# SEpapoulis/ODElib

Measured on AMD Instinct MI355X. Metric: walker-timesteps/sec, 4-state infection ODE, 65536 walkers, 1/2/4/8 MI355X, higher is better.
Workload: dtype f64

## Files before the change

### odelib_amd/csrc/capi.hip

```cpp
#include <hip/hip_runtime.h>

#include <algorithm>
#include <array>
#include <cstdlib>
#include <memory>
#include <mutex>
#include <cmath>
#include <cstdio>
#include <cstring>
#include <new>
#include <string>
#include <vector>

#include "../../include/odelib_amd.h"
#include "aux_kernels.h"
#include "dispatch.h"
#include "launch_plan.h"
#include "rtc.h"

#define OE_BUILTINS(X) \
  X(zero_i) X(one_i) X(two_i) X(chain4) X(chain5) X(chain6) X(chain8) X(chain10) X(chain12) X(chain16) X(chain20) \
  X(chain24) X(chain32)
#define X(NAME) OE_DECLARE_ENTRY(NAME);
OE_BUILTINS(X)
// ... 378 lines not shown
      if (b->p) (void)hipFree(b->p);
    if (c->ev0) (void)hipEventDestroy(c->ev0);
    if (c->ev1) (void)hipEventDestroy(c->ev1);
    if (c->np_stream) {
      (void)hipStreamSynchronize(c->np_stream);
      (void)hipStreamDestroy(c->np_stream);
    }
    for (int k = 0; k < 2; ++k) {
      if (c->ev_np[k]) (void)hipEventDestroy(c->ev_np[k]);
      if (c->ev_mh[k]) (void)hipEventDestroy(c->ev_mh[k]);
    }
    for (auto& m : c->custom)
      for (hipModule_t md : {m->rtc.mod, m->rtc.stiff_mod})
        if (md) (void)hipModuleUnload(md);
    (void)hipStreamDestroy(c->own_stream);
  }
  delete c;
}

const char* oe_last_error(const oe_ctx* c) {
  if (c) return c->err.c_str();
  return g_err.empty() ? "null context" : g_err.c_str();
}

int oe_rtc_check(const char* rhs_body, int32_t n_states, int32_t n_params, const char* arch) {
  if (!rhs_body || n_states < 1 || n_states > 64 || n_params < 1 || n_params > 60)
    return fail(nullptr, OE_ERR_ARG, "oe_rtc_check: bad arguments");
  std::string err;
  if (rtc_build(rhs_body, n_states, n_params, arch ? arch : "gfx950", kRtcExplicit, nullptr, nullptr, err))
    return fail(nullptr, OE_ERR_ARG, err);
  g_err.clear();
  return OE_OK;
}

int oe_model_compile(oe_ctx* c, const char* rhs_body, int32_t n_states, int32_t n_params, int32_t* model_id) {
  if (!c || !c->own_stream) return OE_ERR_STATE;
  if (!rhs_body || !model_id || n_states < 1 || n_states > 64 || n_params < 1 || n_params > 60)
    return fail(c, OE_ERR_ARG, "oe_model_compile: bad arguments");
  for (size_t k = 0; k < c->custom.size(); ++k) {
    const CustomModel& m = *c->custom[k];
    if (m.body == rhs_body && m.entry.S == n_states && m.entry.P == n_params) {
      *model_id = OE_MODEL_CUSTOM + (int32_t)k;
      return OE_OK;
    }
  }
  OE_DEVICE_GUARD(c);
  auto m = std::make_unique<CustomModel>();
  std::string err;
  if (rtc_build(rhs_body, n_states, n_params, c->arch.c_str(), kRtcExplicit, &m->rtc, &m->entry, err))
    return fail(c, OE_ERR_ARG, err);
  m->body = rhs_body;
  m->entry.model_id = OE_MODEL_CUSTOM + (int32_t)c->custom.size();
  m->entry.S = n_states;
  m->entry.P = n_params;
  *model_id = m->entry.model_id;
  c->custom.push_back(std::move(m));
  return OE_OK;
}

int oe_ctx_set_stream(oe_ctx* c, void* s) {
  if (!c || !c->own_stream) return OE_ERR_STATE;
  c->stream = static_cast<hipStream_t>(s);
  return OE_OK;
}

int oe_ctx_use_own_stream(oe_ctx* c) {
  if (!c || !c->own_stream) return OE_ERR_STATE;
  c->stream = c->own_stream;
  return OE_OK;
}

int oe_problem_set(oe_ctx* c, const oe_problem* p) {
  if (!c || !c->own_stream) return OE_ERR_STATE;
  if (!p) return fail(c, OE_ERR_ARG, "oe_problem_set: null problem");
  OE_DEVICE_GUARD(c);
  const Entry* e = nullptr;
  CustomModel* cm = nullptr;
  if (p->model_id >= OE_MODEL_CUSTOM) {
    const size_t k = (size_t)(p->model_id - OE_MODEL_CUSTOM);
    if (k < c->custom.size()) {
      cm = c->custom[k].get();
      e = &cm->entry;
    }
  } else {
    e = find_entry(p->model_id, p->n_states);
  }
  if (!e)
    return fail(c, OE_ERR_UNSUPPORTED, "oe_problem_set: model " + std::to_string(p->model_id) +
                                           " with S=" + std::to_string(p->n_states) +
                                           " is not compiled in");
  if (p->n_states != e->S) return fail(c, OE_ERR_ARG, "oe_problem_set: n_states mismatch");
  const int pmax = e->P + (e->S < 4 ? e->S : 4);
  if (p->n_params < e->P || p->n_params > pmax)
    return fail(c, OE_ERR_ARG, "oe_problem_set: n_params must be in [model P, model P + min(S, 4)]");
  if (p->n_times < 2 || !p->times) return fail(c, OE_ERR_ARG, "oe_problem_set: need >= 2 times");
  for (int i = 1; i < p->n_times; ++i)
    if (!(p->times[i] > p->times[i - 1]))
      return fail(c, OE_ERR_ARG, "oe_problem_set: times must be strictly increasing");
  if (p->method < OE_METHOD_RK4 || p->method > OE_METHOD_BDF)
    return fail(c, OE_ERR_ARG, "oe_problem_set: unknown method");
  if (p->method == OE_METHOD_BDF && e->S > kStiffRegS)
    return fail(c, OE_ERR_UNSUPPORTED, "oe_problem_set: bdf needs n_states <= " + std::to_string(kStiffRegS));
  if (p->method == OE_METHOD_AUTO || p->method == OE_METHOD_ROSENBROCK || p->method == OE_METHOD_BDF) {
    if (cm) {
      if (cm->rtc.stiff == 0) {
        std::string err;
        if (rtc_build(cm->body, e->S, e->P, c->arch.c_str(), kRtcStiff, &cm->rtc, &cm->entry, err)) {
          cm->rtc.stiff = -1;
          cm->rtc.stiff_err = err;
        }
      }
      if (cm->rtc.stiff != 1) return fail(c, OE_ERR_UNSUPPORTED, "oe_problem_set: " + cm->rtc.stiff_err);
    } else if (!e->integrate[p->method][0][0] && !(p->method == OE_METHOD_AUTO && e->integrate_hq[0][0][0])) {
      return fail(c, OE_ERR_UNSUPPORTED, "oe_problem_set: the stiff methods (auto, rosenbrock) need n_states <= " +
                                             std::to_string(kStiffMaxS));
    }
  }
  if (p->method == OE_METHOD_RK4 && p->rk4_substeps < 1)
    return fail(c, OE_ERR_ARG, "oe_problem_set: rk4_substeps must be >= 1");
  if (p->method != OE_METHOD_RK4 &&
      (!(p->rtol > 0.0) || !(p->atol >= 0.0) || p->max_steps < 2))
    return fail(c, OE_ERR_ARG, "oe_problem_set: adaptive methods need rtol > 0, atol >= 0, max_steps >= 2");
  if (p->n_obs < 0) return fail(c, OE_ERR_ARG, "oe_problem_set: n_obs < 0");
  if (p->n_obs > 0 && (!p->obs_tidx || !p->obs_mask || !p->obs_log || !p->obs_logsigma || !p->obs_lin))
    return fail(c, OE_ERR_ARG, "oe_problem_set: observation arrays missing");

  std::vector<Obs> obs_in(p->n_obs);
  const uint64_t valid_mask = (e->S >= 64) ? ~0ull : ((1ull << e->S) - 1ull);
  for (int k = 0; k < p->n_obs; ++k) {
    if (p->obs_tidx[k] < 0 || p->obs_tidx[k] >= p->n_times)
      return fail(c, OE_ERR_ARG, "oe_problem_set: obs_tidx out of range");
    if (p->obs_mask[k] == 0 || (p->obs_mask[k] & ~valid_mask))
      return fail(c, OE_ERR_ARG, "oe_problem_set: obs_mask selects no / unknown states");
    Obs& o = obs_in[k];
    o.tidx = p->obs_tidx[k];
    o.pad = 0;
    o.mask = p->obs_mask[k];
    o.O = p->obs_log[k];
    const double s = p->obs_logsigma[k];
    o.two_s2 = 2.0 * (s * s);
    o.O_lin = p->obs_lin[k];
  }
  std::vector<int32_t> perm(p->n_obs);
  for (int k = 0; k < p->n_obs; ++k) perm[k] = k;
  std::stable_sort(perm.begin(), perm.end(), [&](int32_t a, int32_t b) { return obs_in[a].tidx < obs_in[b].tidx; });
  std::vector<Obs> obs(p->n_obs);
  std::vector<double> c_rec(p->n_obs);
  for (int k = 0; k < p->n_obs; ++k) {
    obs[k] = obs_in[perm[k]];
    c_rec[k] = -(std::log(p->obs_logsigma[perm[k]]) + 0.5 * std::log(2.0 * 3.14159265358979323846));
  }

  const int nsub = p->method == OE_METHOD_RK4 ? p->rk4_substeps : 1;
  std::vector<double> rk4(4 * (size_t)p->n_times);
  for (int i = 1; i < p->n_times; ++i) {
    const double h = (p->times[i] - p->times[i - 1]) / (double)nsub;
    rk4[4 * (i - 1)] = h;
    rk4[4 * (i - 1) + 1] = 0.5 * h;
    rk4[4 * (i - 1) + 2] = h / 6.0;
    rk4[4 * (i - 1) + 3] = p->times[i - 1];
  }
  for (int j = 0; j < 4; ++j) rk4[4 * (size_t)(p->n_times - 1) + j] = rk4[4 * (size_t)(p->n_times - 2) + j];

  OE_HIP(c, hipStreamSynchronize(c->stream));
  if (c->d_times) { OE_HIP(c, hipFree(c->d_times)); c->d_times = nullptr; }
  if (c->d_obs) { OE_HIP(c, hipFree(c->d_obs)); c->d_obs = nullptr; }
  if (c->d_rk4) { OE_HIP(c, hipFree(c->d_rk4)); c->d_rk4 = nullptr; }
  OE_HIP(c, hipMalloc(&c->d_rk4, sizeof(double) * rk4.size()));
  OE_HIP(c, hipMemcpy(c->d_rk4, rk4.data(), sizeof(double) * rk4.size(), hipMemcpyHostToDevice));
  std::vector<double> tg(p->times, p->times + p->n_times);
  tg.insert(tg.end(), oe::kGridWin + 1, HUGE_VAL);
  OE_HIP(c, hipMalloc(&c->d_times, sizeof(double) * tg.size()));
  OE_HIP(c, hipMemcpy(c->d_times, tg.data(), sizeof(double) * tg.size(), hipMemcpyHostToDevice));
  if (p->n_obs > 0) {
    OE_HIP(c, hipMalloc(&c->d_obs, sizeof(Obs) * p->n_obs));
    OE_HIP(c, hipMemcpy(c->d_obs, obs.data(), sizeof(Obs) * p->n_obs, hipMemcpyHostToDevice));
  }
  DevProblem& d = c->dp;
  d.times = c->d_times;
  d.rk4 = c->d_rk4;
  d.obs = c->d_obs;
  d.T = p->n_times;
  d.n_obs = p->n_obs;
  d.P = p->n_params;
  d.substeps = p->method == OE_METHOD_RK4 ? p->rk4_substeps : 1;
  d.rtol = p->rtol;
  d.atol = p->atol;
  d.max_steps = p->max_steps;
  d.pnum = p->pnum;
  d.sstot = p->sstot;
  d.newton_tol = std::fmax(10.0 * 2.220446049250313e-16 / p->rtol, std::fmin(0.03, std::sqrt(p->rtol)));
  c->method = p->method;
  c->entry = e;
  c->has_problem = true;
  c->band_cols = c->band_bins = 0;
  c->waic_on = false;
  c->waic_c = std::move(c_rec);
  c->waic_perm = std::move(perm);
  c->err.clear();
  return OE_OK;
}

int oe_integrate(oe_ctx* c, int64_t W, const double* y0, const double* theta, double* traj,
                 double* chi, double* ssres, int32_t* status, uint32_t flags) {
  if (!c || !c->own_stream) return OE_ERR_STATE;
  if (!c->has_problem) return fail(c, OE_ERR_STATE, "oe_integrate: call oe_problem_set first");
  if (W <= 0 || W > kMaxWalkers) return fail(c, OE_ERR_ARG, "oe_integrate: n_walkers must be in [1, 2^29]");
  if (!y0 || !theta) return fail(c, OE_ERR_ARG, "oe_integrate: y0 and theta are required");
  OE_DEVICE_GUARD(c);
  int rc = OE_OK;
  const Entry* e = c->entry;
  const int S = e->S, P = c->dp.P, T = c->dp.T;
  const bool host = flags & OE_HOST_PTRS;
  const bool nt = flags & OE_NT_STORES;
  if (traj && (int64_t)S * W * 8 >= (int64_t(1) << 32))
    return fail(c, OE_ERR_ARG, "oe_integrate: one trajectory row (S*W*8 bytes) must be < 4 GiB");

  IntegrateArgs ia{};
  ia.W = W;
  if (host) {
    const size_t n_in = (size_t)(S + P) * W;
    const size_t n_traj = traj ? (size_t)T * S * W : 0;
    const size_t n_out = (size_t)2 * W;
    const size_t bytes = sizeof(double) * (n_in + n_traj + n_out) + sizeof(int32_t) * W + 256;
    rc = c->scratch.reserve(c, bytes);
    if (rc) return rc;
    double* base = static_cast<double*>(c->scratch.p);
    double* d_y0 = base;
    double* d_th = d_y0 + (size_t)S * W;
    double* d_traj = traj ? d_th + (size_t)P * W : nullptr;
    double* d_chi = d_th + (size_t)P * W + n_traj;
    double* d_ss = d_chi + W;
    int32_t* d_st = reinterpret_cast<int32_t*>(d_ss + W);
    OE_HIP(c, hipMemcpyAsync(d_y0, y0, sizeof(double) * S * W, hipMemcpyHostToDevice, c->stream));
    OE_HIP(c, hipMemcpyAsync(d_th, theta, sizeof(double) * P * W, hipMemcpyHostToDevice, c->stream));
    ia.y0 = d_y0; ia.theta = d_th; ia.traj = d_traj; ia.chi = d_chi; ia.ssres = d_ss; ia.status = d_st;
  } else {
    ia.y0 = y0; ia.theta = theta; ia.traj = traj; ia.chi = chi; ia.ssres = ssres; ia.status = status;
  }
  const plan::ModelCaps caps = caps_of(e, P);
  plan::IntegratePlan pl =
      plan::plan_integrate(caps, c->method, W, c->n_cu, ia.traj != nullptr, nt, flags, xcd_run_walkers());
  c->dp.obs_c = nullptr;
  if (pl.obs_scratch && c->dp.n_obs > 0) {
    rc = c->obs.reserve(c, sizeof(double) * (size_t)c->dp.n_obs * (size_t)W);
    if (rc) return rc;
    c->dp.obs_c = static_cast<double*>(c->obs.p);
  }
  c->has_last_tune = false;
  if (pl.path == plan::kRk4Traj && (flags & OE_TUNE)) {
    rc = tune_rk4(c, e, caps, ia, nt, flags, pl, &c->last_tune);
    if (rc) return rc;
    plan::shape_rk4_traj(pl, c->last_tune.variant, W, flags, xcd_run_walkers());
    c->has_last_tune = true;
  }
  c->last_variant = pl.variant;
  c->hq_ctl = nullptr;
  ia.half = pl.half;
  ia.xcd_remap = pl.xcd_remap;
  const int tj = ia.traj ? 1 : 0, nj = nt ? 1 : 0;
  const bool wave_stiff = pl.path == plan::kDirectWaveStiff || pl.path == plan::kWaveStiff;
  StiffWaveArgs sa{};
  int32_t* stiff_buf = nullptr;
  if (wave_stiff) {
    rc = c->stiff.reserve(c, sizeof(int32_t) * (size_t)(2 * W + 64));
    if (rc) return rc;
    stiff_buf = static_cast<int32_t*>(c->stiff.p);
    sa.y0 = ia.y0; sa.theta = ia.theta; sa.traj = ia.traj; sa.chi = ia.chi; sa.ssres = ia.ssres; sa.W = W;
    if (!ia.status) ia.status = stiff_buf + 64 + W;
    sa.status = ia.status;
  }
  const bool timing = !(flags & OE_NO_TIMING);
  if (timing) OE_HIP(c, hipEventRecord(c->ev0, c->stream));
  if (pl.path == plan::kHandQueue) {
    HandQ q{};
    rc = ensure_hq(c, W, S, &q);
    if (rc) return rc;
    q.n_waves = (int32_t)pl.grid * (kBlock / 64);
    OE_HIP(c, hipMemsetAsync(q.ctl, 0, 10 * sizeof(int32_t), c->stream));
    hipStream_t bs = c->stream;
    if (pl.beside) {
      OE_HIP(c, hipEventRecord(c->ev_hq[0], c->stream));
      OE_HIP(c, hipStreamWaitEvent(c->hq_stream, c->ev_hq[0], 0));
      bs = c->hq_stream;
    }
    const int bj = pl.beside ? 1 : 0;
    OE_HIP(c, launch(e->integrate_hq[bj][tj][nj], dim3(pl.grid), dim3(pl.block), c->stream, c->dp, ia, q));
    OE_HIP(c, launch(e->bdf_hq[bj][tj][nj], dim3(pl.G), dim3(64), bs, c->dp, ia, q));
    if (pl.beside) {
      OE_HIP(c, hipEventRecord(c->ev_hq[1], c->hq_stream));
      OE_HIP(c, hipStreamWaitEvent(c->stream, c->ev_hq[1], 0));
    }
    c->hq_ctl = q.ctl;
  } else if (pl.path != plan::kWaveStiff) {
    OE_HIP(c, launch_planned(c, e, pl, ia, nt));
  }
  if (wave_stiff) {
    if (pl.path == plan::kDirectWaveStiff) {
      int32_t* count = stiff_buf;
      int32_t* list = stiff_buf + 64;
      OE_HIP(c, hipMemsetAsync(count, 0, sizeof(int32_t), c->stream));
      OE_HIP(c, launch(kernel_of(k_stiff_list), dim3((unsigned)((W + 255) / 256)), dim3(256), c->stream,
                       (const int32_t*)ia.status, W, list, count));
      sa.list = list;
      sa.count = count;
    }
    OE_HIP(c, launch(e->stiff_wave[tj][nj], dim3(pl.wave_grid), dim3(64), c->stream, c->dp, sa));
  }
  OE_HIP(c, hipGetLastError());
  if (timing) OE_HIP(c, hipEventRecord(c->ev1, c->stream));
  c->timed = timing;

  if (host) {
    if (traj)
      OE_HIP(c, hipMemcpyAsync(traj, ia.traj, sizeof(double) * T * S * W, hipMemcpyDeviceToHost, c->stream));
// ... 572 lines not shown
```

### odelib_amd/csrc/ode_kernels.cuh

```cuda
#pragma once
#include <hip/hip_runtime.h>
#include <stdint.h>
#include "models.cuh"

namespace oe {

struct Obs {
  int32_t tidx;
  int32_t pad;
  uint64_t mask;
  double O;
  double two_s2;
  double O_lin;
};

template <class T>
using cptr = const __attribute__((address_space(4))) T*;
template <class T>
__device__ __forceinline__ cptr<T> kconst(const T* p) {
  return (cptr<T>)(p);
}

struct DevProblem {
  const double* times;
// ... 117 lines not shown

typedef unsigned int u32x2 __attribute__((ext_vector_type(2)));
typedef unsigned int u32x4 __attribute__((ext_vector_type(4)));

#ifndef OE_NT_AUX
#define OE_NT_AUX 18
#endif
template <bool NT>
__device__ __forceinline__ void st_row(__amdgpu_buffer_rsrc_t rsrc, uint32_t lane_off, uint32_t s_off, double v) {
  __builtin_amdgcn_raw_buffer_store_b64(__builtin_bit_cast(u32x2, v), rsrc, lane_off, s_off, NT ? OE_NT_AUX : 0);
}

#ifndef OE_TRANSC_CALL
#define OE_TRANSC_CALL 1
#endif
#if OE_TRANSC_CALL
__device__ __attribute__((noinline)) double oe_log(double x) { return log(x); }
__device__ __attribute__((noinline)) double oe_exp(double x) { return exp(x); }
#else
__device__ __forceinline__ double oe_log(double x) { return log(x); }
__device__ __forceinline__ double oe_exp(double x) { return exp(x); }
#endif

template <int S>
__device__ __forceinline__ void check_finite(const double (&y)[S], Acc& a) {
#pragma unroll
  for (int s = 0; s < S; ++s) a.nf = fma(y[s], 0.0, a.nf);
}

template <int S>
__device__ __forceinline__ void track_min(const double (&y)[S], Acc& a) {
  if constexpr (S == 1) {
    a.ymin = min_raw(a.ymin, y[0]);
  } else {
    double m[(S + 1) / 2];
#pragma unroll
    for (int j = 0; j < S / 2; ++j) m[j] = min_raw(y[2 * j], y[2 * j + 1]);
    if constexpr (S % 2) m[S / 2] = y[S - 1];
    double r = m[0];
#pragma unroll
    for (int j = 1; j < (S + 1) / 2; ++j) r = min_raw(r, m[j]);
    a.ymin = min_raw(a.ymin, r);
  }
}

template <int S, bool TRAJ, bool NT>
__device__ __forceinline__ void store_row_at(double* row, const double (&y)[S], int64_t W, uint32_t off,
                                             bool active, Acc& a) {
  track_min<S>(y, a);
  if constexpr (TRAJ) {
    if (active) {
      const uint32_t row_bytes = (uint32_t)(S * W * 8);
      const __amdgpu_buffer_rsrc_t rsrc = __builtin_amdgcn_make_buffer_rsrc((void*)row, 0, row_bytes, 0x00020000);
#pragma unroll
      for (int s = 0; s < S; ++s) st_row<NT>(rsrc, off, (uint32_t)(s * W * 8), y[s]);
    }
  }
}

template <int S, bool TRAJ, bool NT>
__device__ __forceinline__ void store_row(int i, const double (&y)[S], double* __restrict__ traj,
                                          int64_t W, uint32_t off, bool active, Acc& a) {
  store_row_at<S, TRAJ, NT>(TRAJ ? traj + (int64_t)i * S * W : nullptr, y, W, off, active, a);
}

struct ObsTerm { double O, two_s2, O_lin; };
template <class ObsPtr>
__device__ __forceinline__ ObsTerm obs_term(ObsPtr rec) {
  return ObsTerm{rec->O, rec->two_s2, rec->O_lin};
}
template <int S>
__device__ __forceinline__ double masked_sum(const double (&y)[S], uint64_t mask) {
  double c = 0.0;
#pragma unroll
  for (int s = 0; s < S; ++s)
    if ((mask >> s) & 1ull) c = c + y[s];
  return c;
}
template <bool INLINE_LOG = false>
__device__ __forceinline__ double chi_term(const ObsTerm& t, double c) {
  const double d = t.O - (INLINE_LOG ? log(c) : oe_log(c));
  return (d * d) / t.two_s2;
}
template <bool INLINE_LOG = false>
__device__ __forceinline__ void fold_obs(const ObsTerm& t, double c, Acc& a, bool in = true) {
  const double term = chi_term<INLINE_LOG>(t, c);
  if (in && __builtin_isfinite(term)) { a.chi += term; a.nvalid += 1; }
  const double r = c - t.O_lin;
  const double r2 = r * r;
  if (in && !__builtin_isnan(r2)) a.ssres += r2;
}
template <class ObsPtr>
__device__ __forceinline__ int next_observed(const DevProblem& pb, ObsPtr obs, int k) {
  return (k < pb.n_obs) ? obs[k].tidx : 0x7fffffff;
}

template <int S, bool INLINE_LOG = false>
__device__ __forceinline__ void observe(const DevProblem& pb, int i, const double (&y)[S], int& k, Acc& a) {
  const cptr<Obs> obs = kconst(pb.obs);
  if (!(k < pb.n_obs && obs[k].tidx == i)) return;
  check_finite(y, a);
  for (; k < pb.n_obs && obs[k].tidx == i; ++k) {
    const uint64_t mask = obs[k].mask;
    const ObsTerm rec = obs_term(obs + k);
    double c = 0.0;
#pragma unroll
    for (int s = 0; s < S; ++s)
      if ((mask >> s) & 1ull) c = c + y[s];
    fold_obs<INLINE_LOG>(rec, c, a);
  }
}

template <int S>
__device__ __forceinline__ void observe_next(const DevProblem& pb, int i, const double (&y)[S], int& k,
                                             int& nxt, Acc& a) {
  if (i != nxt) return;
  observe<S>(pb, i, y, k, a);
  nxt = next_observed(pb, kconst(pb.obs), k);
}

template <int S, bool TRAJ, bool NT, bool INLINE_LOG = false>
__device__ __forceinline__ void emit(const DevProblem& pb, int i, const double (&y)[S],
                                     double* __restrict__ traj, int64_t W, uint32_t off,
                                     bool active, int& k, Acc& a) {
  store_row<S, TRAJ, NT>(i, y, traj, W, off, active, a);
  observe<S, INLINE_LOG>(pb, i, y, k, a);
}

template <int S, bool TRAJ>
__device__ __forceinline__ bool grid_needs_emit(const DevProblem& pb, int i, int k) {
  if constexpr (TRAJ) return true;
  return k < pb.n_obs && kconst(pb.obs)[k].tidx == i;
}

template <class M, int PMAX>
__device__ __forceinline__ void rk4_step(double (&y)[M::S], double t, double h, double hh, double h6,
                                         const double (&p)[PMAX]) {
  constexpr int S = M::S;
  double k[S], acc[S], yt[S];
  M::rhs(y, t, p, k);
#pragma unroll
  for (int s = 0; s < S; ++s) { acc[s] = k[s]; yt[s] = fma(hh, k[s], y[s]); }
  M::rhs(yt, t + hh, p, k);
#pragma unroll
  for (int s = 0; s < S; ++s) { acc[s] = fma(2.0, k[s], acc[s]); yt[s] = fma(hh, k[s], y[s]); }
  M::rhs(yt, t + hh, p, k);
#pragma unroll
  for (int s = 0; s < S; ++s) { acc[s] = fma(2.0, k[s], acc[s]); yt[s] = fma(h, k[s], y[s]); }
  M::rhs(yt, t + h, p, k);
#pragma unroll
  for (int s = 0; s < S; ++s) { acc[s] = acc[s] + k[s]; y[s] = fma(h6, acc[s], y[s]); }
}

template <class M, int PMAX, bool TRAJ, bool NT>
__device__ __forceinline__ void integrate_rk4(const DevProblem& pb, double (&y)[M::S],
                                              const double (&p)[PMAX], double* traj,
                                              int64_t W, uint32_t off, bool active, Acc& a) {
  constexpr int S = M::S;
  int k = 0;
  emit<S, TRAJ, NT, TRAJ>(pb, 0, y, traj, W, off, active, k, a);
  const int n = pb.substeps;
  const cptr<Obs> obs = kconst(pb.obs);
  cptr<double> tab = kconst(pb.rk4);
  double h = tab[0], hh = tab[1], h6 = tab[2], t = tab[3];
  tab += 4;
  double* trow = TRAJ ? traj + (int64_t)S * W : nullptr;
  auto interval = [&]() {
    const double hn = tab[0], hhn = tab[1], h6n = tab[2], tn = tab[3];
    tab += 4;
    for (int j = 0; j < n; ++j) rk4_step<M, PMAX>(y, t + (double)j * h, h, hh, h6, p);
    h = hn; hh = hhn; h6 = h6n; t = tn;
  };
  int i = 1;
  while (i < pb.T) {
    const int next = (k < pb.n_obs) ? obs[k].tidx : pb.T;
    for (; i < next; ++i) {
      interval();
      if constexpr (TRAJ) {
        store_row_at<S, TRAJ, NT>(trow, y, W, off, active, a);
        trow += S * W;
      }
    }
    if (i < pb.T) {
      interval();
      store_row_at<S, TRAJ, NT>(trow, y, W, off, active, a);
      if constexpr (TRAJ) trow += S * W;
      observe<S, TRAJ>(pb, i, y, k, a);
      ++i;
    }
  }
  check_finite(y, a);
}

namespace dp {
constexpr double c2 = 1.0 / 5, c3 = 3.0 / 10, c4 = 4.0 / 5, c5 = 8.0 / 9;
constexpr double a21 = 1.0 / 5;
constexpr double a31 = 3.0 / 40, a32 = 9.0 / 40;
constexpr double a41 = 44.0 / 45, a42 = -56.0 / 15, a43 = 32.0 / 9;
constexpr double a51 = 19372.0 / 6561, a52 = -25360.0 / 2187, a53 = 64448.0 / 6561,
                 a54 = -212.0 / 729;
constexpr double a61 = 9017.0 / 3168, a62 = -355.0 / 33, a63 = 46732.0 / 5247,
                 a64 = 49.0 / 176, a65 = -5103.0 / 18656;
constexpr double a71 = 35.0 / 384, a73 = 500.0 / 1113, a74 = 125.0 / 192,
                 a75 = -2187.0 / 6784, a76 = 11.0 / 84;
constexpr double e1 = 71.0 / 57600, e3 = -71.0 / 16695, e4 = 71.0 / 1920,
                 e5 = -17253.0 / 339200, e6 = 22.0 / 525, e7 = -1.0 / 40;
constexpr double d1 = -12715105075.0 / 11282082432.0, d3 = 87487479700.0 / 32700410799.0,
                 d4 = -10690763975.0 / 1880347072.0, d5 = 701980252875.0 / 199316789632.0,
                 d6 = -1453857185.0 / 822651844.0, d7 = 69997945.0 / 29380423.0;
constexpr double safe = 0.9, facmin = 0.2, facmax = 10.0;

__device__ const double kTab[36] = {a21, a31, a32, a41, a42, a43, a51, a52, a53, a54, a61, a62, a63, a64, a65,
                                    a71, a73, a74, a75, a76, e1, e3, e4, e5, e6, e7, d1, d3, d4, d5, d6, d7,
                                    c2, c3, c4, c5};
constexpr double kTabC[36] = {a21, a31, a32, a41, a42, a43, a51, a52, a53, a54, a61, a62, a63, a64, a65,
                              a71, a73, a74, a75, a76, e1, e3, e4, e5, e6, e7, d1, d3, d4, d5, d6, d7,
                              c2, c3, c4, c5};
struct Tab {
  double v[36];
};
template <bool VREG, bool MIX = false, bool PIN = false>
__device__ __forceinline__ Tab load_tab() {
  Tab t;
  if constexpr (VREG) {
    int z;
    asm volatile("v_mov_b32 %0, 0" : "=v"(z));
    const double* p = kTab + z;
#pragma unroll
    for (int j = 0; j < 36; ++j) t.v[j] = (MIX && j >= 20) ? kTabC[j] : p[j];
  } else {
    const double c[36] = {a21, a31, a32, a41, a42, a43, a51, a52, a53, a54, a61, a62, a63, a64, a65,
                          a71, a73, a74, a75, a76, e1, e3, e4, e5, e6, e7, d1, d3, d4, d5, d6, d7,
                          c2, c3, c4, c5};
#pragma unroll
    for (int j = 0; j < 36; ++j) {
      if constexpr (PIN) {
        constexpr uint64_t kOne = 1;
        const uint64_t b = __builtin_bit_cast(uint64_t, c[j]);
        uint32_t lo, hi;
        asm volatile("s_mov_b32 %0, %2\n\ts_mov_b32 %1, %3" : "=s"(lo), "=s"(hi)
                     : "i"((uint32_t)(b & 0xffffffffu)), "i"((uint32_t)(b >> 32)));
        (void)kOne;
        t.v[j] = __builtin_bit_cast(double, ((uint64_t)hi << 32) | lo);
      } else {
        t.v[j] = c[j];
      }
    }
  }
  return t;
}

template <int N>
__device__ __forceinline__ double select_r(int r, const double (&c)[N]) {
  static_assert(N >= 1 && N <= 8, "select_r: at most 8 entries");
  auto at = [&](int k) { return c[k < N ? k : N - 1]; };
  const bool b0 = (r & 1) != 0, b1 = (r & 2) != 0, b2 = (r & 4) != 0;
  const double l0 = b0 ? at(1) : at(0), l1 = b0 ? at(3) : at(2);
  const double l2 = b0 ? at(5) : at(4), l3 = b0 ? at(7) : at(6);
  const double m0 = b1 ? l1 : l0, m1 = b1 ? l3 : l2;
  return b2 ? m1 : m0;
}

template <int N>
__device__ __forceinline__ int count_le(const double (&w)[N], double x) {
  int c = 0;
#pragma unroll
  for (int j = 0; j < N; ++j) {
    c += (w[j] <= x) ? 1 : 0;
    asm("" : "+v"(c));
  }
  return c;
}

__device__ __forceinline__ double inv_fifth_root(double x) {
  int e;
  const double m = frexp(x, &e);
  int q = e / 5, r = e % 5;
  if (r < 0) { r += 5; q -= 1; }
  double y = fma(fma(0.2395, m, -0.6505), m, 1.4123);
#pragma unroll
  for (int it = 0; it < 2; ++it) {
    const double y2 = y * y;
    const double y5 = (y2 * y2) * y;
    y = (y * fma(-m, y5, 6.0)) * 0.2;
  }
  constexpr double kC[5] = {1.0, 0.8705505632961241, 0.757858283255199, 0.6597539553864471, 0.5743491774985174};
  return ldexp(select_r(r, kC) * y, -q);
}

constexpr int kFifthBias = 1088;
struct FifthScale {
  double v[2 * kFifthBias];
  constexpr FifthScale() : v() {
    const double c[5] = {1.0, 0.8705505632961241, 0.757858283255199, 0.6597539553864471, 0.5743491774985174};
    for (int j = 0; j < 2 * kFifthBias; ++j) {
      const int e = j - kFifthBias;
      int q = e / 5, r = e % 5;
      if (r < 0) { r += 5; q -= 1; }
      const int be = 1023 - q;
      v[j] = (be > 0 && be < 2047) ? c[r] * __builtin_bit_cast(double, (unsigned long long)be << 52) : 0.0;
    }
  }
};
__device__ const FifthScale kFifthScale{};
__device__ __forceinline__ double inv_fifth_root_uniform(double x, cptr<double> scale) {
  int e;
  const double m = frexp(x, &e);
  e = __builtin_amdgcn_readfirstlane(e);
  const double sc = scale[e + kFifthBias];
  double y = fma(fma(0.2395, m, -0.6505), m, 1.4123);
#pragma unroll
  for (int it = 0; it < 2; ++it) {
    const double y2 = y * y;
    const double y5 = (y2 * y2) * y;
    y = (y * fma(-m, y5, 6.0)) * 0.2;
  }
  return sc * y;
}
}

constexpr int kDpPipeFields = 6;
template <int S>
constexpr int dp_pipe_slots() {
  return (150 * 1024) / (4 * (kDpPipeFields * S * 64 * 8 + 32)) < 8 ? (150 * 1024) / (4 * (kDpPipeFields * S * 64 * 8 + 32)) : 8;
}
template <int S>
struct DpPipe {
  double* ring;
  double* uni;
  volatile int* produced;
  volatile int* consumed;
  int lane, R, n, cons_seen;
};

__device__ __forceinline__ void lds_fence() { asm volatile("s_waitcnt lgkmcnt(0)" ::: "memory"); }

template <int S>
__device__ __forceinline__ void dp_pipe_publish(DpPipe<S>& pp, double t, double tn, double rh, const double (&y)[S],
                                                const double (&ydf)[S], const double (&bsp)[S], const double (&r4)[S],
                                                const double (&r5)[S], const double (&yn)[S]) {
  while (pp.n - pp.cons_seen >= pp.R) {
    pp.cons_seen = *pp.consumed;
    if (pp.n - pp.cons_seen >= pp.R) __builtin_amdgcn_s_sleep(1);
// ... 616 lines not shown
#pragma unroll
  for (int q = 0; q < PMAX; ++q) p[q] = (q < pb.P) ? ia.theta[(int64_t)q * W + w] : 0.0;
#if OE_HQ_TRACE
  const uint64_t t_claim = __builtin_amdgcn_s_memrealtime();
#endif
  if (OE_HQ_PRIO) __builtin_amdgcn_s_setprio(3);
  integrate_bdf_lane<M, PMAX, TRAJ, NT, DREG ? 0 : 64>(pb, y, t, i, k, p, ia.traj, W, w, part, part, a);
#if OE_HQ_TRACE
  {
    const uint64_t t0 = __hip_atomic_load((const uint64_t*)(hq.ctl + 4 + 2), __ATOMIC_RELAXED, __HIP_MEMORY_SCOPE_AGENT);
    const uint64_t t_pend = __hip_atomic_load((const uint64_t*)(hq.ctl + 8), __ATOMIC_RELAXED, __HIP_MEMORY_SCOPE_AGENT);
    a.chi = (double)((int64_t)(t_start - t0) / 100) * 1e5 + (double)((int64_t)(t_pend - t0) / 100);
    a.ssres = (double)((int64_t)(t_claim - t0) / 100) * 1e5 + (double)((__builtin_amdgcn_s_memrealtime() - t_claim) / 100);
    a.nvalid = 1;
  }
#endif
  if (part) {
    if (ia.chi) ia.chi[w] = a.nvalid ? a.chi : __builtin_nan("");
    if (ia.ssres) ia.ssres[w] = a.ssres;
    if (ia.status) ia.status[w] = finish(a);
  }
}

template <class M, bool NT>
__global__ void __launch_bounds__(512) k_integrate_dopri5_piped(const DevProblem pb, const IntegrateArgs ia) {
  constexpr int S = M::S;
  constexpr int PMAX = kPmax<M>;
  constexpr int R = dp_pipe_slots<S>();
  static_assert(R >= 2, "slot ring too small");
  __shared__ double ring[4][R][kDpPipeFields * S * 64];
  __shared__ double uni[4][R][4];
  __shared__ int produced[4], consumed[4];
  __shared__ double ymin_sh[4][64];
  const int wave = threadIdx.x >> 6;
  const int lane = threadIdx.x & 63;
  const int c = wave & 3;
  if (threadIdx.x < 4) { produced[threadIdx.x] = 0; consumed[threadIdx.x] = 0; }
  __syncthreads();
  const int64_t blk = ia.xcd_remap ? xcd_block(blockIdx.x, gridDim.x, ia.xcd_remap) : (int64_t)blockIdx.x;
  const int64_t gw = blk * 256 + c * 64 + lane;
  const bool active = gw < ia.W;
  const int64_t w = active ? gw : ia.W - 1;
  const int64_t W = ia.W;
  const int T = pb.T;
  if (wave < 4) {
    double y[S], p[PMAX];
#pragma unroll
    for (int s = 0; s < S; ++s) y[s] = ia.y0[(int64_t)s * W + w];
#pragma unroll
    for (int j = 0; j < PMAX; ++j) p[j] = (j < pb.P) ? ia.theta[(int64_t)j * W + w] : 0.0;
    Acc a = acc_init();
    DpPipe<S> pp{&ring[c][0][0], &uni[c][0][0], &produced[c], &consumed[c], lane, R, 0, 0};
    integrate_dopri5<M, PMAX, true, NT, false, false, false, true>(pb, y, p, ia.traj, W, (uint32_t)w * 8u, active, a,
                                                                 nullptr, &pp);
    __syncthreads();
    a.ymin = min_raw(a.ymin, ymin_sh[c][lane]);
    if (active) {
      if (ia.chi) ia.chi[w] = a.nvalid ? a.chi : __builtin_nan("");
      if (ia.ssres) ia.ssres[w] = a.ssres;
      if (ia.status) ia.status[w] = finish(a);
    }
  } else {
    const double* times = pb.times;
    const uint32_t off = (uint32_t)w * 8u;
    const uint32_t row_bytes = (uint32_t)(S * W * 8);
    Acc a = acc_init();
    int i = 0;
    for (int n = 0; i < T; ++n) {
      while (*(volatile int*)&produced[c] <= n) __builtin_amdgcn_s_sleep(1);
      asm volatile("" ::: "memory");
      const int slot = n % R;
      const double* f = &ring[c][slot][0] + lane;
      const double t = uni[c][slot][0], tn = uni[c][slot][1], rh = uni[c][slot][2];
      double y[S], ydf[S], bsp[S], r4[S], r5[S], yn[S];
#pragma unroll
      for (int s = 0; s < S; ++s) {
        y[s] = f[(0 * S + s) * 64];
        ydf[s] = f[(1 * S + s) * 64];
        bsp[s] = f[(2 * S + s) * 64];
        r4[s] = f[(3 * S + s) * 64];
        r5[s] = f[(4 * S + s) * 64];
        yn[s] = f[(5 * S + s) * 64];
      }
      lds_fence();
      if (lane == 0) *(volatile int*)&consumed[c] = n + 1;
      double ti = times[i];
      while (ti < tn) {
        const double th = (ti - t) * rh;
        const double th1 = 1.0 - th;
        double yo[S];
#pragma unroll
        for (int s = 0; s < S; ++s)
          yo[s] = fma(th, fma(th1, fma(th, fma(th1, r5[s], r4[s]), bsp[s]), ydf[s]), y[s]);
        store_row_at<S, true, NT>(ia.traj + (int64_t)i * S * W, yo, W, off, active, a);
        ++i;
        ti = times[i];
      }
      if (i < T && ti == tn) {
        store_row_at<S, true, NT>(ia.traj + (int64_t)i * S * W, yn, W, off, active, a);
        ++i;
      }
    }
    (void)row_bytes;
    ymin_sh[c][lane] = a.ymin;
    __syncthreads();
  }
}

constexpr int kPipeWalkers = 256;
#ifndef OE_PIPE_LDS_BYTES
#define OE_PIPE_LDS_BYTES (160 * 1024)
#endif
constexpr int kPipeLdsBytes = OE_PIPE_LDS_BYTES;

template <int S>
constexpr int pipe_rows() { return (kPipeLdsBytes / (2 * S * kPipeWalkers * 8)) > 0 ? (kPipeLdsBytes / (2 * S * kPipeWalkers * 8)) : 1; }

__device__ __forceinline__ void lds_barrier() {
  asm volatile("s_waitcnt lgkmcnt(0)" ::: "memory");
  __builtin_amdgcn_s_barrier();
  asm volatile("" ::: "memory");
}


template <class M, bool NT, int NSW>
__global__ void __launch_bounds__(256 + 64 * NSW) k_integrate_rk4_piped(const DevProblem pb, const IntegrateArgs ia) {
  constexpr int S = M::S;
  constexpr int PMAX = kPmax<M>;
  constexpr int H = pipe_rows<S>();
  static_assert(2 * H * S * kPipeWalkers * 8 <= kPipeLdsBytes, "LDS ring too large");
  __shared__ double pipe_ring[2][H][S][kPipeWalkers];
  auto ring = [&](int half, int h, int s, int b) -> double* { return &pipe_ring[half][h][s][b]; };

  const int64_t W = ia.W;
  const int T = pb.T;
  const int wave = threadIdx.x >> 6;
  const int lane = threadIdx.x & 63;
  const int64_t blk = ia.xcd_remap ? xcd_block(blockIdx.x, gridDim.x, ia.xcd_remap) : (int64_t)blockIdx.x;
  const int64_t base = blk * kPipeWalkers;
  const int nphase = (T + H - 1) / H;

  if (wave < 4) {
    const int b = wave * 64 + lane;
    const int64_t gw = base + b;
    const bool active = gw < W;
    const int64_t w = active ? gw : W - 1;
    double y[S], p[PMAX];
#pragma unroll
    for (int s = 0; s < S; ++s) y[s] = ia.y0[(int64_t)s * W + w];
#pragma unroll
    for (int j = 0; j < PMAX; ++j) p[j] = (j < pb.P) ? ia.theta[(int64_t)j * W + w] : 0.0;
    Acc a = acc_init();
    int k = 0;
    const cptr<double> tab = kconst(pb.rk4);
    const cptr<Obs> obs = kconst(pb.obs);
    const int n = pb.substeps;
    auto put = [&](int half, int h, const double (&v)[S]) {
#pragma unroll
      for (int s = 0; s < S; ++s) *ring(half, h, s, b) = v[s];
#pragma unroll
      for (int s = 0; s < S; ++s) a.ymin = min_raw(a.ymin, v[s]);
    };
    auto interval = [&](int i) {
      const double h = tab[4 * (i - 1)], hh = tab[4 * (i - 1) + 1], h6 = tab[4 * (i - 1) + 2];
      const double t = tab[4 * (i - 1) + 3];
      for (int j = 0; j < n; ++j) rk4_step<M, PMAX>(y, t + (double)j * h, h, hh, h6, p);
    };
    for (int ph = 0; ph <= nphase; ++ph) {
      if (ph < nphase) {
        const int half = ph & 1;
        const int r0 = ph * H;
        const int r1 = (r0 + H < T) ? r0 + H : T;
        int r = r0;
        if (r == 0) {
          put(half, 0, y);
          observe<S, true>(pb, 0, y, k, a);
          ++r;
        }
        while (r < r1) {
          int next = (k < pb.n_obs) ? obs[k].tidx : T;
          if (next > r1) next = r1;
          for (; r < next; ++r) {
            interval(r);
            put(half, r - r0, y);
          }
          if (r < r1) {
            interval(r);
            put(half, r - r0, y);
            observe<S, true>(pb, r, y, k, a);
            ++r;
          }
        }
      }
      lds_barrier();
    }
    check_finite(y, a);
    if (active) {
      if (ia.chi) ia.chi[w] = a.nvalid ? a.chi : __builtin_nan("");
      if (ia.ssres) ia.ssres[w] = a.ssres;
      if (ia.status) ia.status[w] = finish(a);
    }
  } else {
    const int sw = wave - 4;
    constexpr int G = NSW / 2;
    const int sg = sw >> 1;
    const int b = (sw & 1) * 128 + 2 * lane;
    const bool active = base + b < W;
    const uint32_t off = (uint32_t)(base + b) * 8u;
    const uint32_t row_bytes = (uint32_t)(S * W * 8);
    for (int ph = 0; ph <= nphase; ++ph) {
      if (ph >= 1) {
        const int half = (ph - 1) & 1;
        const int r0 = (ph - 1) * H;
        const int r1 = (r0 + H < T) ? r0 + H : T;
        for (int r = r0; r < r1; ++r) {
          const __amdgpu_buffer_rsrc_t rsrc =
              __builtin_amdgcn_make_buffer_rsrc((void*)(ia.traj + (int64_t)r * S * W), 0, row_bytes, 0x00020000);
#pragma unroll
          for (int s0 = 0; s0 < S; s0 += G) {
            const int s = s0 + sg;
            if (G > 1 && s >= S) break;
            const u32x4 v = *reinterpret_cast<const u32x4*>(ring(half, r - r0, s, b));
            if (active)
              __builtin_amdgcn_raw_buffer_store_b128(v, rsrc, off, (uint32_t)(s * W * 8), NT ? OE_NT_AUX : 0);
          }
        }
      }
      lds_barrier();
    }
  }
}

}
#include "stiff_wave.cuh"
#include "split.cuh"
#include "mh.cuh"
```

Baseline: 197.0 billion.

## Prefetch RK4 step-table rows with scalar vector loads ahead of integration

Replaces per-interval scalar loads of the RK4 step table (h, h/2, h/6, t) with s_load_dwordx16 inline asm that fetches two rows at a time, issued one interval ahead so the constant-memory latency overlaps the RK4 arithmetic. When substeps==1, a lean path unrolls four intervals per iteration and also drops the substep loop. The chi-only path is split from the trajectory path and now batches observation-free runs. The host pads the table with look-ahead rows so over-reads stay in bounds. Inline asm with manual waitcnt adds fragility around compiler scheduling and register constraints.

Measured after the change: 197.3 billion, median of 6. No clear change (+0.2%).

```diff
diff --git a/odelib_amd/csrc/capi.hip b/odelib_amd/csrc/capi.hip
--- a/odelib_amd/csrc/capi.hip
+++ b/odelib_amd/csrc/capi.hip
@@ -554,7 +554,8 @@
   }
 
   const int nsub = p->method == OE_METHOD_RK4 ? p->rk4_substeps : 1;
-  std::vector<double> rk4(4 * (size_t)p->n_times);
+  const size_t n_iv = (size_t)p->n_times - 1;
+  std::vector<double> rk4(oe::kRk4RowDoubles * oe::rk4_table_rows(p->n_times));
   for (int i = 1; i < p->n_times; ++i) {
     const double h = (p->times[i] - p->times[i - 1]) / (double)nsub;
     rk4[4 * (i - 1)] = h;
@@ -562,7 +563,9 @@
     rk4[4 * (i - 1) + 2] = h / 6.0;
     rk4[4 * (i - 1) + 3] = p->times[i - 1];
   }
-  for (int j = 0; j < 4; ++j) rk4[4 * (size_t)(p->n_times - 1) + j] = rk4[4 * (size_t)(p->n_times - 2) + j];
+  for (size_t r = n_iv; r < oe::rk4_table_rows(p->n_times); ++r)
+    for (int j = 0; j < 4; ++j) rk4[4 * r + j] = rk4[4 * (n_iv - 1) + j];
+  static_assert(oe::kRk4RowDoubles == 4, "a row is h, h/2, h/6, t");
 
   OE_HIP(c, hipStreamSynchronize(c->stream));
   if (c->d_times) { OE_HIP(c, hipFree(c->d_times)); c->d_times = nullptr; }
diff --git a/odelib_amd/csrc/ode_kernels.cuh b/odelib_amd/csrc/ode_kernels.cuh
--- a/odelib_amd/csrc/ode_kernels.cuh
+++ b/odelib_amd/csrc/ode_kernels.cuh
@@ -293,19 +293,107 @@
   for (int s = 0; s < S; ++s) { acc[s] = acc[s] + k[s]; y[s] = fma(h6, acc[s], y[s]); }
 }
 
-template <class M, int PMAX, bool TRAJ, bool NT>
-__device__ __forceinline__ void integrate_rk4(const DevProblem& pb, double (&y)[M::S],
-                                              const double (&p)[PMAX], double* traj,
-                                              int64_t W, uint32_t off, bool active, Acc& a) {
+typedef double f64x8 __attribute__((ext_vector_type(8)));
+constexpr int kRk4RowDoubles = 4;
+constexpr int kRk4RowsPerLoad = 2;
+constexpr int kRk4LookAhead = 2;
+static_assert(kRk4LookAhead >= kRk4RowsPerLoad,
+              "the stream loads kRk4RowsPerLoad rows starting at the row after the last interval's");
+constexpr size_t rk4_table_rows(int T) { return (size_t)(T - 1) + kRk4LookAhead; }
+
+template <int ROW_OFF>
+__device__ __forceinline__ f64x8 rk4_rows_issue(cptr<double> at, double& y0) {
+  f64x8 v;
+  asm volatile("s_load_dwordx16 %0, %2, %3" : "=&s"(v), "+v"(y0) : "s"(at), "n"(ROW_OFF * kRk4RowDoubles * 8));
+  return v;
+}
+__device__ __forceinline__ void rk4_rows_wait(f64x8& v, double& y0) {
+  asm volatile("s_waitcnt lgkmcnt(0)" : "+s"(v), "+v"(y0));
+}
+template <class M, int PMAX, int R>
+__device__ __forceinline__ void rk4_interval(double (&y)[M::S], const f64x8& rows, int n, const double (&p)[PMAX]) {
+  const double h = rows[4 * R], hh = rows[4 * R + 1], h6 = rows[4 * R + 2], t = rows[4 * R + 3];
+  for (int j = 0; j < n; ++j) rk4_step<M, PMAX>(y, t + (double)j * h, h, hh, h6, p);
+}
+template <class M, int PMAX, int R>
+__device__ __forceinline__ void rk4_interval1(double (&y)[M::S], const f64x8& rows, const double (&p)[PMAX]) {
+  const double h = rows[4 * R], hh = rows[4 * R + 1], h6 = rows[4 * R + 2], t = rows[4 * R + 3];
+  rk4_step<M, PMAX>(y, t + 0.0 * h, h, hh, h6, p);
+}
+
+template <class M, int PMAX>
+struct Rk4Rows {
+  cptr<double> tab;
+  f64x8 cur;
+  const int n;
+  const bool lean;
+  __device__ __forceinline__ Rk4Rows(const DevProblem& pb, double (&y)[M::S])
+      : tab(kconst(pb.rk4)), n(pb.substeps), lean(pb.substeps == 1) {
+    cur = rk4_rows_issue<0>(tab, y[0]);
+    rk4_rows_wait(cur, y[0]);
+  }
+  template <class After>
+  __device__ __forceinline__ void run(double (&y)[M::S], const double (&p)[PMAX], int m, After after) {
+    int j = 0;
+    if (lean) {
+      for (int q = m >> 2; q > 0; --q, j += 4) {
+        f64x8 nxt = rk4_rows_issue<2>(tab, y[0]);
+        rk4_interval1<M, PMAX, 0>(y, cur, p);
+        after(j);
+        rk4_interval1<M, PMAX, 1>(y, cur, p);
+        after(j + 1);
+        rk4_rows_wait(nxt, y[0]);
+        cur = rk4_rows_issue<4>(tab, y[0]);
+        tab += 4 * kRk4RowDoubles;
+        rk4_interval1<M, PMAX, 0>(y, nxt, p);
+        after(j + 2);
+        rk4_interval1<M, PMAX, 1>(y, nxt, p);
+        after(j + 3);
+        rk4_rows_wait(cur, y[0]);
+      }
+    }
+    for (; j < m; ++j) {
+      f64x8 nxt = rk4_rows_issue<1>(tab, y[0]);
+      tab += kRk4RowDoubles;
+      rk4_interval<M, PMAX, 0>(y, cur, n, p);
+      after(j);
+      rk4_rows_wait(nxt, y[0]);
+      cur = nxt;
+    }
+  }
+};
+
+template <class M, int PMAX>
+__device__ __forceinline__ void integrate_rk4_chi(const DevProblem& pb, double (&y)[M::S],
+                                                  const double (&p)[PMAX], int& k, Acc& a) {
   constexpr int S = M::S;
-  int k = 0;
-  emit<S, TRAJ, NT, TRAJ>(pb, 0, y, traj, W, off, active, k, a);
+  const int T = pb.T;
+  const cptr<Obs> obs = kconst(pb.obs);
+  Rk4Rows<M, PMAX> rows(pb, y);
+  int i = 1;
+  while (i < T) {
+    const bool seen = k < pb.n_obs;
+    const int stop = seen ? obs[k].tidx : T - 1;
+    rows.run(y, p, stop - i + 1, [](int) {});
+    i = stop + 1;
+    if (seen) {
+      track_min<S>(y, a);
+      observe<S, false>(pb, stop, y, k, a);
+    }
+  }
+}
+
+template <class M, int PMAX, bool NT>
+__device__ __forceinline__ void integrate_rk4_traj(const DevProblem& pb, double (&y)[M::S],
+                                                   const double (&p)[PMAX], double* traj,
+                                                   int64_t W, uint32_t off, bool active, int& k, Acc& a) {
+  constexpr int S = M::S;
   const int n = pb.substeps;
   const cptr<Obs> obs = kconst(pb.obs);
   cptr<double> tab = kconst(pb.rk4);
   double h = tab[0], hh = tab[1], h6 = tab[2], t = tab[3];
   tab += 4;
-  double* trow = TRAJ ? traj + (int64_t)S * W : nullptr;
+  double* trow = traj + (int64_t)S * W;
   auto interval = [&]() {
     const double hn = tab[0], hhn = tab[1], h6n = tab[2], tn = tab[3];
     tab += 4;
@@ -317,19 +405,29 @@
     const int next = (k < pb.n_obs) ? obs[k].tidx : pb.T;
     for (; i < next; ++i) {
       interval();
-      if constexpr (TRAJ) {
-        store_row_at<S, TRAJ, NT>(trow, y, W, off, active, a);
-        trow += S * W;
-      }
+      store_row_at<S, true, NT>(trow, y, W, off, active, a);
+      trow += S * W;
     }
     if (i < pb.T) {
       interval();
-      store_row_at<S, TRAJ, NT>(trow, y, W, off, active, a);
-      if constexpr (TRAJ) trow += S * W;
-      observe<S, TRAJ>(pb, i, y, k, a);
+      store_row_at<S, true, NT>(trow, y, W, off, active, a);
+      trow += S * W;
+      observe<S, true>(pb, i, y, k, a);
       ++i;
     }
   }
+}
+
+template <class M, int PMAX, bool TRAJ, bool NT>
+__device__ __forceinline__ void integrate_rk4(const DevProblem& pb, double (&y)[M::S],
+                                              const double (&p)[PMAX], double* traj,
+                                              int64_t W, uint32_t off, bool active, Acc& a) {
+  int k = 0;
+  emit<M::S, TRAJ, NT, TRAJ>(pb, 0, y, traj, W, off, active, k, a);
+  if constexpr (TRAJ)
+    integrate_rk4_traj<M, PMAX, NT>(pb, y, p, traj, W, off, active, k, a);
+  else
+    integrate_rk4_chi<M, PMAX>(pb, y, p, k, a);
   check_finite(y, a);
 }
 
@@ -1252,19 +1350,13 @@
     for (int j = 0; j < PMAX; ++j) p[j] = (j < pb.P) ? ia.theta[(int64_t)j * W + w] : 0.0;
     Acc a = acc_init();
     int k = 0;
-    const cptr<double> tab = kconst(pb.rk4);
     const cptr<Obs> obs = kconst(pb.obs);
-    const int n = pb.substeps;
+    Rk4Rows<M, PMAX> rows(pb, y);
     auto put = [&](int half, int h, const double (&v)[S]) {
 #pragma unroll
       for (int s = 0; s < S; ++s) *ring(half, h, s, b) = v[s];
 #pragma unroll
       for (int s = 0; s < S; ++s) a.ymin = min_raw(a.ymin, v[s]);
-    };
-    auto interval = [&](int i) {
-      const double h = tab[4 * (i - 1)], hh = tab[4 * (i - 1) + 1], h6 = tab[4 * (i - 1) + 2];
-      const double t = tab[4 * (i - 1) + 3];
-      for (int j = 0; j < n; ++j) rk4_step<M, PMAX>(y, t + (double)j * h, h, hh, h6, p);
     };
     for (int ph = 0; ph <= nphase; ++ph) {
       if (ph < nphase) {
@@ -1278,18 +1370,13 @@
           ++r;
         }
         while (r < r1) {
-          int next = (k < pb.n_obs) ? obs[k].tidx : T;
-          if (next > r1) next = r1;
-          for (; r < next; ++r) {
-            interval(r);
-            put(half, r - r0, y);
-          }
-          if (r < r1) {
-            interval(r);
-            put(half, r - r0, y);
-            observe<S, true>(pb, r, y, k, a);
-            ++r;
-          }
+          const int next = (k < pb.n_obs) ? obs[k].tidx : T;
+          const bool seen = next < r1;
+          const int m = (seen ? next + 1 : r1) - r;
+          const int h0 = r - r0;
+          rows.run(y, p, m, [&](int j) { put(half, h0 + j, y); });
+          r += m;
+          if (seen) observe<S, true>(pb, next, y, k, a);
         }
       }
       lds_barrier();
```
